# NVIDIA/makani

Hardware: NVIDIA H100
Metric: SFNO-block fwd+bwd samples/sec (higher is better)
Workload: dtype tf32

## Files before the change

### makani_b200/csrc/dft.cu

```cuda
#include "umma_common.cuh"
#include "wgmma_tf32.cuh"
#include "dft_math.cuh"
#include <cmath>
#include <cstdlib>
#include <vector>

namespace b200sht {

int umma_available();

constexpr int kDftMaxHalf = 95;
constexpr int kDftSynWorkers = 10;
constexpr int kDftSynThreads = 32 * (kDftSynWorkers + 2);
constexpr int kDftSynStages = 4;
__host__ __device__ constexpr int dft_out_box(int N2) {
  int d = N2 < 32 ? N2 : 32;
  while (N2 % d != 0) --d;
  return 8 * d;
}

struct DftTables {
  float* et;
  float* eb;
  float2* tw;
  float* zeros;
  int N2, half, M2, nkb;
};

bool dft_shape_ok(int nlon, int mmax) {
  if (nlon % 8 != 0) return false;
  const int N2 = nlon / 8;
  return N2 >= 2 && N2 / 2 <= kDftMaxHalf && (mmax + 7) / 8 <= 32 && mmax <= nlon / 2 + 1;
}

__global__ void dft_tables_kernel(float* et, float* eb, float2* tw, int N2, int half, int M2, int nkb, int nlon) {
  const int i = blockIdx.x * blockDim.x + threadIdx.x;
  if (i < 2 * 128 * 32) {
    const int m2 = i % 32, row = i / 32, p = (row >> 3) & 1, j2 = 8 * (row >> 4) + (row & 7);
    float v = 0.f;
    if (j2 <= half && m2 < M2) {
      const long long t = ((long long)m2 * j2) % N2;
      const double ang = 2.0 * M_PI * (double)t / (double)N2;
      v = tf32_rn((float)(p == 0 ? cos(ang) : sin(ang)));
    }
    et[i] = v;
  }
  if (i < nkb * 2 * 32 * 32) {
    const int jl = i % 32, m2 = (i / 32) % 32, p = (i / 1024) % 2, kb = i / 2048;
    const int j2 = kb * 32 + jl;
    float v = 0.f;
    if (j2 <= half && m2 < M2) {
      const long long t = ((long long)m2 * j2) % N2;
      const double ang = 2.0 * M_PI * (double)t / (double)N2;
      v = tf32_rn((float)(p == 0 ? cos(ang) : sin(ang)));
      if (2 * j2 == N2) v *= 0.5f;
    }
    eb[i] = v;
  }
  if (i < 8 * N2) {
    const int j2 = i % N2, c = i / N2;
    const double ang = 2.0 * M_PI * (double)(c * j2) / (double)nlon;
    tw[i] = make_float2((float)cos(ang), (float)sin(ang));
  }
}

int dft_plan_init(Plan* pl) {
  pl->dft_state = nullptr;
  if (!umma_available()) return -1;
  if (!dft_shape_ok(pl->nlon, pl->mmax)) return -1;
  DftTables* t = new DftTables();
  t->N2 = pl->nlon / 8; t->half = t->N2 / 2; t->M2 = (pl->mmax + 7) / 8;
  t->nkb = (t->half + 1 + 31) / 32;
  t->et = nullptr; t->eb = nullptr; t->tw = nullptr; t->zeros = nullptr;
  const size_t neb = (size_t)t->nkb * 2 * 32 * 32;
  cudaError_t e = cudaMalloc(&t->et, sizeof(float) * 2 * 128 * 32);
  if (e == cudaSuccess) e = cudaMalloc(&t->eb, sizeof(float) * neb);
  if (e == cudaSuccess) e = cudaMalloc(&t->tw, sizeof(float2) * 8 * t->N2);
  if (e == cudaSuccess) e = cudaMalloc(&t->zeros, sizeof(float) * 8 * t->N2);
  if (e == cudaSuccess) e = cudaMemset(t->zeros, 0, sizeof(float) * 8 * t->N2);
  if (e == cudaSuccess) {
    const int n = 8192 > 8 * t->N2 ? 8192 : 8 * t->N2;
    dft_tables_kernel<<<(n + 255) / 256, 256>>>(t->et, t->eb, t->tw, t->N2, t->half, t->M2, t->nkb, pl->nlon);
    e = cudaGetLastError();
    if (e == cudaSuccess) e = cudaStreamSynchronize(0);
  }
  if (e != cudaSuccess) {
    cudaFree(t->et); cudaFree(t->eb); cudaFree(t->tw); cudaFree(t->zeros);
    delete t;
    return -1;
  }
  pl->dft_state = t;
  return 0;
}

void dft_plan_destroy(Plan* pl) {
  DftTables* t = static_cast<DftTables*>(pl->dft_state);
  if (!t) return;
  cudaFree(t->et); cudaFree(t->eb); cudaFree(t->tw); cudaFree(t->zeros);
  delete t;
  pl->dft_state = nullptr;
}

static bool dft_enabled() {
  static const int on = [] { const char* e = getenv("B200SHT_DFT"); return e ? atoi(e) : 1; }();
  return on != 0;
}
bool dft_usable(const Plan* pl) { return pl->dft_state != nullptr && dft_enabled(); }

static unsigned long long* g_dft_prof = nullptr;
static unsigned long long* dft_prof_buffer() {
  static const int on = [] { const char* e = getenv("B200SHT_DFT_PROF"); return e ? atoi(e) : 0; }();
  if (!on) return nullptr;
  if (!g_dft_prof) {
    if (cudaMalloc(&g_dft_prof, 16 * sizeof(unsigned long long)) != cudaSuccess) { g_dft_prof = nullptr; return nullptr; }
    cudaMemset(g_dft_prof, 0, 16 * sizeof(unsigned long long));
  }
  return g_dft_prof;
}
int dft_profile_read(unsigned long long* out16) {
  if (!g_dft_prof) { for (int i = 0; i < 16; ++i) out16[i] = 0; return 0; }
  B200_CHECK_CUDA(cudaDeviceSynchronize());
  B200_CHECK_CUDA(cudaMemcpy(out16, g_dft_prof, 16 * sizeof(unsigned long long), cudaMemcpyDeviceToHost));
  B200_CHECK_CUDA(cudaMemset(g_dft_prof, 0, 16 * sizeof(unsigned long long)));
  return 0;
}
#ifdef B200SHT_DFT_PROFILE
constexpr bool kDftProfile = true;
#else
constexpr bool kDftProfile = false;
#endif
__device__ __forceinline__ void prof_wait(unsigned long long* prof, int slot, uint64_t* bar, uint32_t parity, bool lead) {
  if (!kDftProfile || prof == nullptr) { mbar_wait(bar, parity); return; }
  const long long t0 = clock64();
  mbar_wait(bar, parity);
  if (lead) atomicAdd(prof + slot, (unsigned long long)(clock64() - t0));
}
__device__ __forceinline__ void prof_wait_nocall(unsigned long long* prof, int slot, uint64_t* bar, uint32_t parity, bool lead) {
  if (!kDftProfile || prof == nullptr) { mbar_wait_nocall(bar, parity); return; }
  const long long t0 = clock64();
  mbar_wait_nocall(bar, parity);
  if (lead) atomicAdd(prof + slot, (unsigned long long)(clock64() - t0));
}

static int make_tmap_out(CUtensorMap* tm, void* base, bool bf16, int nlon, int nlat, long long rows, int ow) {
  TmapKey key;
  memset(&key, 0, sizeof(key));
  key.base = base; key.rank = 3; key.kind = bf16 ? 7 : 6;
  key.dims[0] = nlon; key.dims[1] = nlat; key.dims[2] = rows; key.box[0] = ow;
  int slot = 0;
  if (tmap_lookup(key, tm, &slot)) return 0;
  PFN_encodeTiled enc = get_encode();
  if (!enc) { set_error("cuTensorMapEncodeTiled is unavailable"); return B200SHT_ERR_UNSUPPORTED; }
  static thread_local bool ctx_bound = false;
  if (!ctx_bound) { cudaFree(nullptr); ctx_bound = true; }
  const int es = bf16 ? 2 : 4;
  cuuint64_t gd[3] = {(cuuint64_t)nlon, (cuuint64_t)nlat, (cuuint64_t)rows};
  cuuint64_t gst[2] = {(cuuint64_t)nlon * es, (cuuint64_t)nlon * nlat * es};
  cuuint32_t bx[3] = {(cuuint32_t)ow, 8, 1}, el[3] = {1, 1, 1};
  if (gst[0] % 16 != 0 || (reinterpret_cast<uintptr_t>(base) & 15) != 0 || (ow * es) % 16 != 0) {
    set_error("tensor map (output): base / row pitch / box row not 16-byte aligned");
    return B200SHT_ERR_INVALID;
  }
  CUresult r = enc(tm, bf16 ? CU_TENSOR_MAP_DATA_TYPE_BFLOAT16 : CU_TENSOR_MAP_DATA_TYPE_FLOAT32, 3, base, gd, gst, bx, el,
                   CU_TENSOR_MAP_INTERLEAVE_NONE, CU_TENSOR_MAP_SWIZZLE_NONE, CU_TENSOR_MAP_L2_PROMOTION_L2_256B, CU_TENSOR_MAP_FLOAT_OOB_FILL_NONE);
  if (r != CUDA_SUCCESS) { set_error("cuTensorMapEncodeTiled (output) failed (%d)", (int)r); return B200SHT_ERR_CUDA; }
  tmap_store(key, tm, slot);
  return 0;
}

template <typename T> __device__ __forceinline__ void st_out(T* p, float v);
template <> __device__ __forceinline__ void st_out<float>(float* p, float v) { *p = v; }
template <> __device__ __forceinline__ void st_out<__nv_bfloat16>(__nv_bfloat16* p, float v) { *p = __float2bfloat16_rn(v); }
template <typename T> __device__ __forceinline__ uint32_t ld_raw(const T* p);
template <> __device__ __forceinline__ uint32_t ld_raw<float>(const float* p) { return __float_as_uint(__ldg(p)); }
template <> __device__ __forceinline__ uint32_t ld_raw<__nv_bfloat16>(const __nv_bfloat16* p) { return (uint32_t)__ldg(reinterpret_cast<const unsigned short*>(p)); }

#ifndef B200_DFT_TF32_MODE
#define B200_DFT_TF32_MODE 2
#endif
constexpr float kTruncComp = 1.0f + 0.0009765625f / 3.0f;
__device__ __forceinline__ float tf32_operand(float v) {
#if B200_DFT_TF32_MODE == 0
  return tf32_rn(v);
#elif B200_DFT_TF32_MODE == 1
  return __uint_as_float((__float_as_uint(v) + 0x1000u) & 0xffffe000u);
#else
  return v;
#endif
}
__device__ __forceinline__ float tf32_operand_unscaled(float v) {
#if B200_DFT_TF32_MODE == 2
  return v * kTruncComp;
#else
  return tf32_operand(v);
#endif
}

__device__ __forceinline__ pr pr_operand(pr v) { return make_pr(tf32_operand(v.v.x), tf32_operand(v.v.y)); }
__device__ __forceinline__ pr pr_operand_unscaled(pr v) {
#if B200_DFT_TF32_MODE == 2
  return rmul(v, kTruncComp);
#else
  return pr_operand(v);
#endif
}

template <typename T> __device__ __forceinline__ float ld_in(const T* p);
template <> __device__ __forceinline__ float ld_in<float>(const float* p) { return __ldg(p); }
template <> __device__ __forceinline__ float ld_in<__nv_bfloat16>(const __nv_bfloat16* p) {
  return __uint_as_float((uint32_t)__ldg(reinterpret_cast<const unsigned short*>(p)) << 16);
}

struct DftSynParams {
  alignas(64) CUtensorMap tmZ;
  alignas(64) CUtensorMap tmE;
  alignas(64) CUtensorMap tmY;
  const float* Z;
  const float2* tw;
  const float* rowscale;
  const float* bias;
  unsigned long long* prof;
  int R, C, nlat, nlon, kp, mmax, N2, half, M2, mode, ntiles, ktiles, has_nyq, ow;
};

template <typename T>
__global__ void __launch_bounds__(kDftSynThreads, 1) dft_synthesis_kernel(const __grid_constant__ DftSynParams p) {
  extern __shared__ uint8_t smem_raw[];
  __shared__ unsigned long long prof_s[16];
  unsigned long long* const prof = (kDftProfile && p.prof) ? prof_s : nullptr;
  if (kDftProfile && threadIdx.x < 16) prof_s[threadIdx.x] = 0;
  const uint32_t raw = smem_u32(smem_raw);
  const uint32_t base = (raw + 1023u) & ~1023u;
  uint8_t* gbase = smem_raw + (base - raw);
  const int N2 = p.N2;
  const int nlon = 8 * N2;
  const int ow = p.ow;
  const uint32_t obytes = (8u * nlon * sizeof(T) + 1023u) & ~1023u;
  const uint32_t sA = base, sB = base + 32768, sO = sB + kDftSynStages * 16384;
  T* const outS = reinterpret_cast<T*>(gbase + (sO - base));
  float2* tws = reinterpret_cast<float2*>(gbase + (sO - base) + 2 * obytes);
  int* oofs = reinterpret_cast<int*>(reinterpret_cast<uint8_t*>(tws) + ((8 * N2 * 8 + 15) & ~15));
  uint64_t* bars = reinterpret_cast<uint64_t*>(reinterpret_cast<uint8_t*>(oofs) + 8 * N2 * 4);
  uint64_t* full = bars;
  uint64_t* empty = full + kDftSynStages;
  uint64_t* e_full = empty + kDftSynStages;
  uint64_t* staged = e_full + 1;
  uint64_t* ofree = staged + 2;

  const int warp = __shfl_sync(0xffffffffu, (int)(threadIdx.x >> 5), 0), lane = threadIdx.x & 31;
  pdl_trigger();
  const int nblk = (p.half + 8) / 8;
  const int nwork = kDftSynWorkers < 2 * nblk ? kDftSynWorkers : 2 * nblk;
  const bool is_tma = (warp == kDftSynWorkers), is_store = (warp == kDftSynWorkers + 1);

  if (threadIdx.x == 0) {
    for (int s = 0; s < kDftSynStages; ++s) { mbar_init(&full[s], 1); mbar_init(&empty[s], nblk); }
    mbar_init(e_full, 1);
    for (int b = 0; b < 2; ++b) { mbar_init(&staged[b], 32 * nblk); mbar_init(&ofree[b], 1); }
    fence_barrier_init();
    prefetch_tmap(&p.tmZ);
    prefetch_tmap(&p.tmE);
    prefetch_tmap(&p.tmY);
  }
  for (int i = threadIdx.x; i < 8 * p.N2; i += blockDim.x) tws[i] = p.tw[i];
  for (int i = threadIdx.x; i < 8 * N2; i += blockDim.x) {
    const int j = N2 * (i & 7) + (i >> 3);
    oofs[i] = (j / ow) * 8 * ow + j % ow;
  }
  __syncthreads();
  const long long t_cta0 = (kDftProfile && p.prof && threadIdx.x == 0) ? clock64() : 0;
  pdl_wait();

  if (is_tma) {
    if (lane == 0) {
      mbar_expect_tx(e_full, 32768);
      tma_load_2d(sA, &p.tmE, e_full, 0, 0);
      tma_load_2d(sA + 16384, &p.tmE, e_full, 0, 128);
      int n = 0;
      for (int ti = blockIdx.x; ti < p.ntiles; ti += gridDim.x, ++n) {
        const int s = n % kDftSynStages, it = n / kDftSynStages;
        if (it > 0) prof_wait(prof, 8, &empty[s], (it - 1) & 1, true);
        mbar_expect_tx(&full[s], 16384);
        const uint32_t st = sB + s * 16384;
        tma_load_5d(st, &p.tmZ, &full[s], 0, 0, 0, 0, ti);
        tma_load_5d(st + 4096, &p.tmZ, &full[s], 0, 1, 0, 0, ti);
        tma_load_5d(st + 8192, &p.tmZ, &full[s], 0, 0, 0, 1, ti);
        tma_load_5d(st + 12288, &p.tmZ, &full[s], 0, 1, 0, 1, ti);
      }
    }
    __syncwarp();
  } else if (is_store) {
    if (lane == 0) {
      int n = 0;
      for (int ti = blockIdx.x; ti < p.ntiles; ti += gridDim.x, ++n) {
        const int b = n & 1;
        prof_wait(prof, 11, &staged[b], (n >> 1) & 1, true);
        const int r = ti / p.ktiles, k0 = (ti - r * p.ktiles) * 8;
        if (k0 < p.nlat)
          for (int bx = 0; bx * ow < nlon; ++bx) tma_store_3d(&p.tmY, sO + b * obytes + bx * 8 * ow * (uint32_t)sizeof(T), bx * ow, k0, r);
        bulk_commit();
        bulk_wait_read0();
        mbar_arrive(&ofree[b]);
      }
      bulk_wait0();
    }
    __syncwarp();
  } else {
    const int kpi = lane & 3;
    const bool n2odd = (N2 & 1) != 0;
    const float smul = p.mode == 0 ? 2.f : 1.f;
    const int nyq_m = nlon / 2;
    const uint8_t* const gE = gbase;
    uint32_t zoff[2][4];
#pragma unroll
    for (int h = 0; h < 2; ++h)
#pragma unroll
      for (int cc = 0; cc < 4; ++cc) zoff[h][cc] = swz128((uint32_t)((kpi + 4 * h) * 128 + (8 * cc + (lane >> 2)) * 4));
    mbar_wait(e_full, 0);
    for (int task = warp; warp < nwork; task += nwork) {
      const int n = task / nblk, blk = task - n * nblk;
      const int ti = blockIdx.x + n * gridDim.x;
      if (ti >= p.ntiles) break;
      const int r = ti / p.ktiles, k0 = (ti - r * p.ktiles) * 8;
      const int ka = k0 + 2 * kpi;
      const int s = n % kDftSynStages, it = n / kDftSynStages;
      float rsa = 1.f, rsb = 1.f, z0a = 0.f, z0b = 0.f, zna = 0.f, znb = 0.f;
      if (p.mode == 1) {
        const float2 rs = *reinterpret_cast<const float2*>(p.rowscale + ka);
        rsa = rs.x; rsb = rs.y;
      } else {
        const float* zt = p.Z + (size_t)ti * 2 * p.M2 * 64 + 2 * kpi;
        const float2 z0 = *reinterpret_cast<const float2*>(zt);
        z0a = z0.x; z0b = z0.y;
        if (p.has_nyq) {
          const float2 zn = *reinterpret_cast<const float2*>(zt + (nyq_m >> 3) * 64 + (nyq_m & 7) * 8);
          zna = zn.x; znb = zn.y;
        }
      }
      const float bias = p.bias ? __ldg(p.bias + r % p.C) : 0.f;
      const pr sc = make_pr(smul * rsa, smul * rsb);
      const pr off_e = make_pr(bias - rsa * (z0a + zna), bias - rsb * (z0b + znb));
      const pr off_o = make_pr(bias - rsa * (z0a - zna), bias - rsb * (z0b - znb));
      prof_wait(prof, 9, &full[s], it & 1, lane == 0);
      if (prof && lane == 0) atomicAdd(prof + 13, 1ull);
      float acc[2][8][4];
#pragma unroll
      for (int a = 0; a < 2; ++a)
#pragma unroll
        for (int c = 0; c < 8; ++c) acc[a][c][0] = acc[a][c][1] = acc[a][c][2] = acc[a][c][3] = 0.f;
      {
        const uint8_t* const zs = gbase + 32768 + (size_t)s * 16384;
#pragma unroll
        for (int kk = 0; kk < 32; kk += 8) {
          uint32_t fa[4];
          frag_a<false>(gE, 16 * blk, kk, fa);
#pragma unroll
          for (int c = 0; c < 8; ++c) {
            const uint8_t* const zc = zs + (c >> 2) * 4096 + kk * 128;
            const uint32_t zr[2] = {*reinterpret_cast<const uint32_t*>(zc + zoff[0][c & 3]), *reinterpret_cast<const uint32_t*>(zc + zoff[1][c & 3])};
            const uint32_t zi[2] = {*reinterpret_cast<const uint32_t*>(zc + 8192 + zoff[0][c & 3]),
                                    *reinterpret_cast<const uint32_t*>(zc + 8192 + zoff[1][c & 3])};
            mma_tf32(acc[0][c], fa, zr);
            mma_tf32(acc[1][c], fa, zi);
          }
        }
      }
      __syncwarp();
      if (lane == 0) mbar_arrive(&empty[s]);
      {
        const int j2 = 8 * blk + (lane >> 2);
        const bool valid = j2 <= p.half;
        const bool paired = valid && j2 != 0 && 2 * j2 != N2;
        const int jp = N2 - j2;
        float2 tw[8], tp[8];
        tw[0] = make_float2(1.f, 0.f);
#pragma unroll
        for (int c = 1; c < 8; ++c) tw[c] = valid ? tws[c * N2 + j2] : make_float2(1.f, 0.f);
        dft_partner_twiddles(tw, tp);
        T* const ob = outS + (size_t)(n & 1) * (obytes / sizeof(T)) + 2 * kpi * ow;
        if (n >= 2) prof_wait(prof, 10, &ofree[n & 1], ((n >> 1) - 1) & 1, lane == 0);
        {
          pr vr[8], vi[8], x[8];
#pragma unroll
          for (int c = 0; c < 8; ++c) {
            vr[c] = make_pr(acc[0][c][0], acc[0][c][1]) - make_pr(acc[1][c][2], acc[1][c][3]);
            vi[c] = make_pr(acc[0][c][2], acc[0][c][3]) + make_pr(acc[1][c][0], acc[1][c][1]);
          }
          dft_syn_radix8<pr>(vr, vi, tw, x);
          const pr o0 = (j2 & 1) ? off_o : off_e, o1 = (j2 & 1) ? off_e : off_o;
          const int4* const op = reinterpret_cast<const int4*>(oofs + 8 * (valid ? j2 : 0));
          const int4 oa = op[0], ob4 = op[1];
          const int of[8] = {oa.x, oa.y, oa.z, oa.w, ob4.x, ob4.y, ob4.z, ob4.w};
#pragma unroll
          for (int j1 = 0; j1 < 8; ++j1) {
            const pr o = rfma(x[j1], sc, (n2odd && (j1 & 1)) ? o1 : o0);
            if (valid) { st_out<T>(ob + of[j1], o.v.x); st_out<T>(ob + of[j1] + ow, o.v.y); }
          }
        }
        {
          pr vr[8], vi[8], x[8];
#pragma unroll
          for (int c = 0; c < 8; ++c) {
            vr[c] = make_pr(acc[0][c][0], acc[0][c][1]) + make_pr(acc[1][c][2], acc[1][c][3]);
            vi[c] = make_pr(acc[1][c][0], acc[1][c][1]) - make_pr(acc[0][c][2], acc[0][c][3]);
          }
          dft_syn_radix8<pr>(vr, vi, tp, x);
          const pr o0 = (jp & 1) ? off_o : off_e, o1 = (jp & 1) ? off_e : off_o;
          const int4* const op = reinterpret_cast<const int4*>(oofs + 8 * (paired ? jp : 0));
          const int4 oa = op[0], ob4 = op[1];
          const int of[8] = {oa.x, oa.y, oa.z, oa.w, ob4.x, ob4.y, ob4.z, ob4.w};
#pragma unroll
          for (int j1 = 0; j1 < 8; ++j1) {
            const pr o = rfma(x[j1], sc, (n2odd && (j1 & 1)) ? o1 : o0);
            if (paired) { st_out<T>(ob + of[j1], o.v.x); st_out<T>(ob + of[j1] + ow, o.v.y); }
          }
        }
        fence_proxy_async();
        mbar_arrive(&staged[n & 1]);
      }
    }
  }
  __syncthreads();
  if (kDftProfile && p.prof && threadIdx.x == 0) prof_s[12] = (unsigned long long)(clock64() - t_cta0);
  if (kDftProfile) __syncthreads();
  if (kDftProfile && p.prof && threadIdx.x < 16) atomicAdd(p.prof + threadIdx.x, prof_s[threadIdx.x]);
}

int dft_synthesis(const Plan* pl, const float* Z, void* y, int dtype, int B, int C, const float* bias, int mode, cudaStream_t st) {
  const DftTables* t = static_cast<const DftTables*>(pl->dft_state);
  B200_REQUIRE(t != nullptr, "dft_synthesis: plan has no DFT tables");
  const int R = B * C;
  DftSynParams p;
  memset(&p, 0, sizeof(p));
  p.Z = Z; p.tw = t->tw; p.rowscale = pl->d_rowscale; p.bias = bias; p.prof = dft_prof_buffer();
  p.R = R; p.C = C; p.nlat = pl->nlat; p.nlon = pl->nlon; p.kp = pl->kp; p.mmax = pl->mmax;
  p.N2 = t->N2; p.half = t->half; p.mode = mode;
  p.ktiles = pl->kp / 8; p.ntiles = R * p.ktiles;
  p.has_nyq = (pl->mmax == pl->nlon / 2 + 1) ? 1 : 0;
  p.M2 = t->M2;
  {
    long long d[5] = {32, 2, t->M2, 2, (long long)R * (pl->kp / 8)}, s[5] = {1, 32, 64, (long long)t->M2 * 64, 2ll * t->M2 * 64};
    int bx[5] = {32, 1, 32, 1, 1};
    int rc = make_tmap(&p.tmZ, Z, 5, d, s, bx);
    if (rc) return rc;
  }
  {
    long long d[2] = {32, 256}, s[2] = {1, 32};
    int bx[2] = {32, 128};
    int rc = make_tmap(&p.tmE, t->et, 2, d, s, bx);
    if (rc) return rc;
  }
  const bool bf16 = (dtype == B200SHT_BF16);
  p.ow = dft_out_box(t->N2);
  {
    int rc = make_tmap_out(&p.tmY, y, bf16, pl->nlon, pl->nlat, R, p.ow);
    if (rc) return rc;
  }
  const size_t obytes = (8 * (size_t)pl->nlon * (bf16 ? 2 : 4) + 1023) & ~(size_t)1023;
  const size_t smem = 1024 + 32768 + (size_t)kDftSynStages * 16384 + 2 * obytes + ((8 * (size_t)t->N2 * 8 + 15) & ~(size_t)15) +
                      8 * (size_t)t->N2 * 4 + (2 * kDftSynStages + 5) * 8;
  const int sms = usable_sms(pl->sm_count > 0 ? pl->sm_count : 132);
  const int ctas = p.ntiles < sms ? p.ntiles : sms;
#define B200_LAUNCH_SYN(TT)                                                                                          \
  do {                                                                                                                \
    struct Tag {};                                                                                                    \
    B200_CHECK_CUDA((ensure_dynamic_smem<Tag>(dft_synthesis_kernel<TT>, smem)));                                     \
    B200_CHECK_CUDA(launch_pdl(dft_synthesis_kernel<TT>, dim3(ctas), dim3(kDftSynThreads), smem, st, p));            \
  } while (0)
  if (bf16) { B200_LAUNCH_SYN(__nv_bfloat16); } else { B200_LAUNCH_SYN(float); }
#undef B200_LAUNCH_SYN
  B200_CHECK_LAUNCH();
  return 0;
}

__host__ __device__ constexpr int dft_box_group(int N2, int es) { return (N2 * es) % 16 == 0 ? 1 : (2 * N2 * es) % 16 == 0 ? 2 : (4 * N2 * es) % 16 == 0 ? 4 : 8; }

static int make_tmap_segments(CUtensorMap* tm, const void* base, bool bf16, int nlon, int gs, long long rows, int box_cols) {
  TmapKey key;
  memset(&key, 0, sizeof(key));
  key.base = base; key.rank = 3; key.kind = bf16 ? 5 : 4;
  key.dims[0] = nlon; key.dims[1] = gs; key.dims[2] = rows; key.box[0] = box_cols;
  int slot = 0;
  if (tmap_lookup(key, tm, &slot)) return 0;
  PFN_encodeTiled enc = get_encode();
  if (!enc) { set_error("cuTensorMapEncodeTiled is unavailable"); return B200SHT_ERR_UNSUPPORTED; }
  static thread_local bool ctx_bound = false;
  if (!ctx_bound) { cudaFree(nullptr); ctx_bound = true; }
  const int es = bf16 ? 2 : 4, N2 = nlon / 8;
  cuuint64_t gd[3] = {(cuuint64_t)gs * N2, (cuuint64_t)(8 / gs), (cuuint64_t)rows};
  cuuint64_t gst[2] = {(cuuint64_t)gs * N2 * es, (cuuint64_t)nlon * es};
  cuuint32_t bx[3] = {(cuuint32_t)box_cols, (cuuint32_t)(8 / gs), 16}, el[3] = {1, 1, 1};
  if (gst[0] % 16 != 0 || gst[1] % 16 != 0 || (reinterpret_cast<uintptr_t>(base) & 15) != 0 || (box_cols * es) % 16 != 0) {
    set_error("tensor map (segments): base / pitch / box row not 16-byte aligned");
    return B200SHT_ERR_INVALID;
  }
  CUresult r = enc(tm, bf16 ? CU_TENSOR_MAP_DATA_TYPE_BFLOAT16 : CU_TENSOR_MAP_DATA_TYPE_FLOAT32, 3, const_cast<void*>(base), gd, gst, bx, el,
                   CU_TENSOR_MAP_INTERLEAVE_NONE, CU_TENSOR_MAP_SWIZZLE_NONE, CU_TENSOR_MAP_L2_PROMOTION_L2_256B, CU_TENSOR_MAP_FLOAT_OOB_FILL_NONE);
  if (r != CUDA_SUCCESS) { set_error("cuTensorMapEncodeTiled (segments) failed (%d)", (int)r); return B200SHT_ERR_CUDA; }
  tmap_store(key, tm, slot);
  return 0;
}

constexpr int kDftAnaStages = 2;
constexpr int kDftAnaMma = 8, kDftAnaLoader = 8, kDftAnaProd0 = 9, kDftAnaThreads = 544;

struct DftAnaParams {
  alignas(64) CUtensorMap tmB;
  alignas(64) CUtensorMap tmXc;
  alignas(64) CUtensorMap tmXp;
  float* X;
  const float2* tw;
  const float* rowscale;
  unsigned long long* prof;
  int R, nlat, nlon, kp, mmax, N2, half, M2, nkb, mode, ntiles, ktiles, nraw, gs;
};

template <typename T, int N2T>
__global__ void __launch_bounds__(kDftAnaThreads, 1) dft_analysis_kernel(const __grid_constant__ DftAnaParams p) {
  extern __shared__ uint8_t smem_raw[];
  __shared__ unsigned long long prof_s[16];
  unsigned long long* const prof = (kDftProfile && p.prof) ? prof_s : nullptr;
  if (kDftProfile && threadIdx.x < 16) prof_s[threadIdx.x] = 0;
  const uint32_t raw = smem_u32(smem_raw);
  const uint32_t base = (raw + 1023u) & ~1023u;
  uint8_t* gbase = smem_raw + (base - raw);
  constexpr int kAl = 16 / (int)sizeof(T);
  constexpr int kWc = (sizeof(T) == 2) ? 40 : 32, kWp = (sizeof(T) == 2) ? 40 : 36;
  constexpr uint32_t kColBytes = 16u * kWc * sizeof(T), kParBytes = 16u * kWp * sizeof(T);
  constexpr uint32_t kRawBytes = 8u * (kColBytes + kParBytes);
  const uint32_t oB = 0, oA = 3 * 8192, oR = oA + kDftAnaStages * 65536, oT = oR + (uint32_t)p.nraw * kRawBytes, oBar = oT + 3 * 7 * 32 * 8;
  const uint32_t sBm = base + oB, sAr = base + oA, sRaw = base + oR;
  uint8_t* gA = gbase + oA;
  const uint8_t* gR = gbase + oR;
  float2* twS = reinterpret_cast<float2*>(gbase + oT);
  uint64_t* full = reinterpret_cast<uint64_t*>(gbase + oBar);
  uint64_t* empty = full + kDftAnaStages;
  uint64_t* raw_full = empty + kDftAnaStages;
  uint64_t* raw_empty = raw_full + 4;
  uint64_t* b_full = raw_empty + 4;

  const int warp = __shfl_sync(0xffffffffu, (int)(threadIdx.x >> 5), 0), lane = threadIdx.x & 31;
  pdl_trigger();
  const int nkb = p.nkb;
  const int N2 = N2T > 0 ? N2T : p.N2;
  const int gs = N2T > 0 ? dft_box_group(N2T, (int)sizeof(T)) : p.gs;
  for (int i = threadIdx.x; i < nkb * 7 * 32; i += blockDim.x) {
    const int ln = i & 31, c = (i >> 5) % 7 + 1, kb = i / 224;
    const int j2 = 32 * kb + ln;
    float2 w = (j2 <= p.half) ? p.tw[c * N2 + j2] : make_float2(1.f, 0.f);
#if B200_DFT_TF32_MODE == 2
    w.x *= kTruncComp; w.y *= kTruncComp;
#endif
    twS[i] = w;
  }
  if (threadIdx.x == 0) {
    for (int s = 0; s < kDftAnaStages; ++s) { mbar_init(&full[s], 8 * 32); mbar_init(&empty[s], kDftAnaMma); }
    for (int s = 0; s < p.nraw; ++s) { mbar_init(&raw_full[s], 1); mbar_init(&raw_empty[s], 8); }
    mbar_init(b_full, 1);
    fence_barrier_init();
    prefetch_tmap(&p.tmB);
    prefetch_tmap(&p.tmXc);
    prefetch_tmap(&p.tmXp);
  }
  for (int i = threadIdx.x; i < kDftAnaStages * 2 * 512; i += blockDim.x) {
    const int st = i >> 10, pl = (i >> 9) & 1, off = i & 511;
    reinterpret_cast<float*>(gA + (size_t)st * 65536)[(pl ? 12288 : 4096) + off] = 0.f;
  }
  fence_proxy_async();
  __syncthreads();
  const long long t_cta0 = (kDftProfile && p.prof && threadIdx.x == 0) ? clock64() : 0;
  pdl_wait();

  if (warp == kDftAnaLoader) {
    if (lane == 0) {
      mbar_expect_tx(b_full, (uint32_t)nkb * 8192);
      for (int kb = 0; kb < nkb; ++kb) {
        tma_load_2d(sBm + kb * 8192, &p.tmB, b_full, 0, kb * 64);
        tma_load_2d(sBm + kb * 8192 + 4096, &p.tmB, b_full, 0, kb * 64 + 32);
      }
      int n = 0;
      for (int ti = blockIdx.x; ti < p.ntiles; ti += gridDim.x, ++n) {
        const int r = ti / p.ktiles, row0 = r * p.nlat + (ti - r * p.ktiles) * 16;
        for (int kb = 0; kb < nkb; ++kb) {
          const int g = n * nkb + kb, rs = g % p.nraw, it = g / p.nraw;
          if (it > 0) prof_wait_nocall(prof, 2, &raw_empty[rs], (it - 1) & 1, true);
          mbar_expect_tx(&raw_full[rs], kRawBytes);
          const uint32_t dst = sRaw + rs * kRawBytes;
#pragma unroll
          for (int gm = 0; gm < 8; ++gm) {
            if (gm >= gs) break;
            const int sc = N2 * gm + 32 * kb, sp = N2 * gm + N2 - 32 * kb - 31;
            tma_load_3d(dst + gm * (8 / gs) * kColBytes, &p.tmXc, &raw_full[rs], (sc / kAl) * kAl, 0, row0);
            tma_load_3d(dst + 8 * kColBytes + gm * (8 / gs) * kParBytes, &p.tmXp, &raw_full[rs], sp < 0 ? 0 : (sp / kAl) * kAl, 0, row0);
          }
        }
      }
    }
    __syncwarp();
  } else if (warp < kDftAnaMma) {
    const size_t plane = (size_t)p.R * p.kp;
    const int c = warp, gq = lane >> 2, q = lane & 3;
    const uint32_t aw = sAr + (uint32_t)(warp >> 2) * 8192;
    mbar_wait_nocall(b_full, 0);
    int n = 0;
    for (int ti = blockIdx.x; ti < p.ntiles; ti += gridDim.x, ++n) {
      const int r = ti / p.ktiles, k0 = (ti - r * p.ktiles) * 16;
      float acc[8][4];
      int prev = 0;
      for (int kb = 0; kb < nkb; ++kb) {
        const int g = n * nkb + kb, s = g % kDftAnaStages, it = g / kDftAnaStages;
        prof_wait_nocall(prof, 3, &full[s], it & 1, lane == 0);
        const uint32_t a0 = aw + (uint32_t)s * 65536;
        const uint64_t d_er = wgmma_desc_kmajor(a0), d_ei = wgmma_desc_kmajor(a0 + 16384);
        const uint64_t d_or = wgmma_desc_kmajor(a0 + 32768), d_oi = wgmma_desc_kmajor(a0 + 49152);
        const uint64_t d_c = wgmma_desc_kmajor(sBm + kb * 8192), d_s = wgmma_desc_kmajor(sBm + kb * 8192 + 4096);
        wgmma_fence();
#pragma unroll
        for (int k = 0; k < 4; ++k) {
          const int sd = (kb > 0 || k > 0) ? 1 : 0;
          wgmma_tf32<32, 1, 8, 0>(acc, d_er + 2 * k, d_c + 2 * k, sd);
          wgmma_tf32<32, 1, 8, 4>(acc, d_ei + 2 * k, d_c + 2 * k, sd);
          wgmma_tf32<32, 1, 8, 0>(acc, d_oi + 2 * k, d_s + 2 * k, 1);
          wgmma_tf32<32, -1, 8, 4>(acc, d_or + 2 * k, d_s + 2 * k, 1);
        }
        wgmma_commit();
        wgmma_wait<1>();
        if (kb > 0 && lane == 0) mbar_arrive(&empty[prev]);
        prev = s;
      }
      wgmma_wait<0>();
      wgmma_fence_operands(acc);
      if (lane == 0) mbar_arrive(&empty[prev]);
      if (prof && lane == 0) atomicAdd(prof + 5, 1ull);
#pragma unroll
      for (int h = 0; h < 2; ++h) {
        const int k = k0 + gq + 8 * h;
        if (k >= p.kp) continue;
        const float rs = (p.mode == 0) ? ((k < p.nlat) ? __ldg(p.rowscale + k) : 0.f) : 1.f;
        float* xb = p.X + (size_t)r * p.kp + k;
#pragma unroll
        for (int j = 0; j < 4; ++j)
#pragma unroll
          for (int e = 0; e < 2; ++e) {
            const int m = c + 8 * (8 * j + 2 * q + e);
            if (m >= p.mmax) continue;
            const float sc = ((p.mode == 0) ? rs : ((m == 0 || 2 * m == p.nlon) ? 1.f : 2.f)) * kTruncComp;
            float* dst = xb + (size_t)m * 2 * plane;
            dst[0] = __uint_as_float(__float_as_uint(acc[j][2 * h + e] * sc) & 0xffffe000u);
            dst[plane] = __uint_as_float(__float_as_uint(acc[4 + j][2 * h + e] * sc) & 0xffffe000u);
          }
      }
    }
  } else {
    const int pw = warp - kDftAnaProd0;
    constexpr int nprod = kDftAnaThreads / 32 - kDftAnaProd0;
    static_assert(nprod >= 1 && nprod <= 8, "every producer warp must take an item of every K-block (8 items each)");
    constexpr bool kBf16 = (sizeof(T) == 2);
    const T* const rawS = reinterpret_cast<const T*>(gR);
    int n = 0;
    for (int ti = blockIdx.x; ti < p.ntiles; ti += gridDim.x, ++n) {
      const int r = ti / p.ktiles, kt16 = (ti - r * p.ktiles) * 16;
      for (int item = pw; item < 8 * nkb; item += nprod) {
        const int kb = item >> 3, q = item & 7;
        const int k0 = kt16 + 2 * q;
        const int g = n * nkb + kb;
        const int j2 = 32 * kb + lane;
        const int rs = g % p.nraw;
        prof_wait_nocall(prof, 0, &raw_full[rs], (g / p.nraw) & 1, lane == 0);
        if (prof && lane == 0) atomicAdd(prof + 7, 1ull);
        const T* const rb = rawS + (size_t)rs * (kRawBytes / sizeof(T));
        pr xa[8], xb[8];
#pragma unroll
        for (int j1 = 0; j1 < 8; ++j1) {
          const int gm = j1 % gs, ga = j1 / gs, npb = 8 / gs;
          const int sc = N2 * gm + 32 * kb, sp = N2 * gm + N2 - 32 * kb - 31;
          const int ic = sc - (sc / kAl) * kAl + lane;
          int ip = N2 * gm + N2 - j2 - (sp < 0 ? 0 : (sp / kAl) * kAl);
          ip = ip < 0 ? 0 : (ip > kWp - 1 ? kWp - 1 : ip);
          const T* b0 = rb + gm * (16 * npb * kWc) + (2 * q) * (npb * kWc) + ga * kWc;
          const T* b1 = rb + 8 * (16 * kWc) + gm * (16 * npb * kWp) + (2 * q) * (npb * kWp) + ga * kWp;
          const int rowc = npb * kWc, rowp = npb * kWp;
          if constexpr (kBf16) {
            xa[j1] = make_pr(__uint_as_float((uint32_t)reinterpret_cast<const unsigned short*>(b0)[ic] << 16),
                             __uint_as_float((uint32_t)reinterpret_cast<const unsigned short*>(b0)[rowc + ic] << 16));
            xb[j1] = make_pr(__uint_as_float((uint32_t)reinterpret_cast<const unsigned short*>(b1)[ip] << 16),
                             __uint_as_float((uint32_t)reinterpret_cast<const unsigned short*>(b1)[rowp + ip] << 16));
          } else {
            xa[j1] = make_pr(reinterpret_cast<const float*>(b0)[ic], reinterpret_cast<const float*>(b0)[rowc + ic]);
            xb[j1] = make_pr(reinterpret_cast<const float*>(b1)[ip], reinterpret_cast<const float*>(b1)[rowp + ip]);
          }
        }
        if (kb == 0) {
#pragma unroll
          for (int j1 = 0; j1 < 8; ++j1) xb[j1] = (lane == 0) ? make_pr(0.f, 0.f) : xb[j1];
        }
        if (k0 + 1 >= p.nlat) {
          const bool row0ok = k0 < p.nlat;
#pragma unroll
          for (int j1 = 0; j1 < 8; ++j1) {
            xa[j1] = make_pr(row0ok ? xa[j1].v.x : 0.f, 0.f);
            xb[j1] = make_pr(row0ok ? xb[j1].v.x : 0.f, 0.f);
          }
        }
        pr er[8], ei[8], br[8], bi[8];
        float2 tw[8], tp[8];
        tw[0] = make_float2(1.f, 0.f);
        const float2* const twl = twS + kb * 224 + lane;
#pragma unroll
        for (int c = 1; c < 8; ++c) tw[c] = twl[(c - 1) * 32];
        dft_partner_twiddles(tw, tp);
        dft_ana_radix8<pr>(xa, tw, er, ei);
        dft_ana_radix8<pr>(xb, tp, br, bi);
        __syncwarp();
        if (lane == 0) mbar_arrive(&raw_empty[rs]);
        const int s = g % kDftAnaStages, it = g / kDftAnaStages;
        if (it > 0) prof_wait_nocall(prof, 1, &empty[s], (it - 1) & 1, lane == 0);
        float* const stg = reinterpret_cast<float*>(gA + (size_t)s * 65536);
        const int kr0 = 2 * q;
        float* const d0 = stg + kr0 * 32 + ((((lane >> 2) ^ (kr0 & 7)) << 2) | (lane & 3));
        float* const d1 = stg + (kr0 + 1) * 32 + ((((lane >> 2) ^ ((kr0 + 1) & 7)) << 2) | (lane & 3));
#pragma unroll
        for (int c = 0; c < 8; ++c) {
          pr ye_r = er[c] + br[c], yo_r = er[c] - br[c];
          if (c == 0) { ye_r = pr_operand_unscaled(ye_r); yo_r = pr_operand_unscaled(yo_r); }
          else { ye_r = pr_operand(ye_r); yo_r = pr_operand(yo_r); }
          d0[c * 512] = ye_r.v.x; d1[c * 512] = ye_r.v.y;
          d0[8192 + c * 512] = yo_r.v.x; d1[8192 + c * 512] = yo_r.v.y;
          if (c != 0) {
            const pr ye_i = pr_operand(ei[c] + bi[c]), yo_i = pr_operand(ei[c] - bi[c]);
            d0[4096 + c * 512] = ye_i.v.x; d1[4096 + c * 512] = ye_i.v.y;
            d0[12288 + c * 512] = yo_i.v.x; d1[12288 + c * 512] = yo_i.v.y;
          }
        }
        fence_proxy_async();
        mbar_arrive(&full[s]);
      }
    }
  }
  __syncthreads();
  if (kDftProfile && p.prof && threadIdx.x == 0) prof_s[6] = (unsigned long long)(clock64() - t_cta0);
  if (kDftProfile) __syncthreads();
  if (kDftProfile && p.prof && threadIdx.x < 16) atomicAdd(p.prof + threadIdx.x, prof_s[threadIdx.x]);
}

int dft_analysis(const Plan* pl, const void* x, int dtype, int B, int C, float* X, int mode, cudaStream_t st) {
  const DftTables* t = static_cast<const DftTables*>(pl->dft_state);
  B200_REQUIRE(t != nullptr, "dft_analysis: plan has no DFT tables");
  const int R = B * C;
  DftAnaParams p;
  memset(&p, 0, sizeof(p));
  p.X = X; p.tw = t->tw; p.rowscale = pl->d_rowscale; p.prof = dft_prof_buffer();
  p.R = R; p.nlat = pl->nlat; p.nlon = pl->nlon; p.kp = pl->kp; p.mmax = pl->mmax;
  p.N2 = t->N2; p.half = t->half; p.M2 = t->M2; p.nkb = t->nkb; p.mode = mode;
  p.ktiles = (pl->kp + 15) / 16; p.ntiles = R * p.ktiles;
  const bool bf16 = (dtype == B200SHT_BF16);
  p.nraw = bf16 ? 3 : 2;
  {
    long long d[2] = {32, (long long)t->nkb * 64}, s[2] = {1, 32};
    int bx[2] = {32, 32};
    int rc = make_tmap(&p.tmB, t->eb, 2, d, s, bx);
    if (rc) return rc;
  }
  B200_REQUIRE(bf16 || t->N2 % 4 == 0, "dft_analysis: fp32 input needs nlon %% 32 == 0 (16-byte aligned TMA boxes)");
// ... 116 lines not shown
```

Measured before the change: 853.6.

## Pre-permute DFT synthesis operands in shared memory for vectorized MMA fragment loads

The E matrix is now loaded by plain global reads into a fragment-ordered shared layout, and the TMA warp rearranges each staged Z tile so workers fetch MMA B fragments with single 16-byte loads. A new per-stage 'ready' barrier sits between the TMA arrival and the worker compute. Twiddles are packed as float4, output offsets are precomputed in bytes with paired bf16 conversion, and integer divides are replaced by magic-number fast division. The aim is fewer shared-memory load instructions and less index arithmetic in the inner loop. In exchange the producer warp does extra shuffling work and there is one more synchronisation stage per tile.

```diff
diff --git a/makani_b200/csrc/dft.cu b/makani_b200/csrc/dft.cu
--- a/makani_b200/csrc/dft.cu
+++ b/makani_b200/csrc/dft.cu
@@ -17,6 +17,20 @@
   int d = N2 < 32 ? N2 : 32;
   while (N2 % d != 0) --d;
   return 8 * d;
+}
+
+struct FastDiv {
+  uint32_t m, s;
+  int d;
+  __device__ __forceinline__ int div(int n) const { return (int)((__umulhi((uint32_t)n, m) + (uint32_t)n) >> s); }
+};
+static FastDiv make_fastdiv(int d) {
+  FastDiv f;
+  f.d = d;
+  f.s = 0;
+  while ((1ll << f.s) < d) ++f.s;
+  f.m = (uint32_t)((((1ull << 32) * ((1ull << f.s) - (unsigned long long)d)) / (unsigned long long)d) + 1);
+  return f;
 }
 
 struct DftTables {
@@ -168,9 +182,16 @@
   return 0;
 }
 
-template <typename T> __device__ __forceinline__ void st_out(T* p, float v);
-template <> __device__ __forceinline__ void st_out<float>(float* p, float v) { *p = v; }
-template <> __device__ __forceinline__ void st_out<__nv_bfloat16>(__nv_bfloat16* p, float v) { *p = __float2bfloat16_rn(v); }
+template <typename T> __device__ __forceinline__ void st_out2(uint8_t* p0, uint8_t* p1, float a, float b);
+template <> __device__ __forceinline__ void st_out2<float>(uint8_t* p0, uint8_t* p1, float a, float b) {
+  *reinterpret_cast<float*>(p0) = a;
+  *reinterpret_cast<float*>(p1) = b;
+}
+template <> __device__ __forceinline__ void st_out2<__nv_bfloat16>(uint8_t* p0, uint8_t* p1, float a, float b) {
+  const __nv_bfloat162 v = __floats2bfloat162_rn(a, b);
+  *reinterpret_cast<__nv_bfloat16*>(p0) = v.x;
+  *reinterpret_cast<__nv_bfloat16*>(p1) = v.y;
+}
 template <typename T> __device__ __forceinline__ uint32_t ld_raw(const T* p);
 template <> __device__ __forceinline__ uint32_t ld_raw<float>(const float* p) { return __float_as_uint(__ldg(p)); }
 template <> __device__ __forceinline__ uint32_t ld_raw<__nv_bfloat16>(const __nv_bfloat16* p) { return (uint32_t)__ldg(reinterpret_cast<const unsigned short*>(p)); }
@@ -213,15 +234,19 @@
 
 struct DftSynParams {
   alignas(64) CUtensorMap tmZ;
-  alignas(64) CUtensorMap tmE;
   alignas(64) CUtensorMap tmY;
   const float* Z;
+  const float* et;
   const float2* tw;
   const float* rowscale;
   const float* bias;
   unsigned long long* prof;
-  int R, C, nlat, nlon, kp, mmax, N2, half, M2, mode, ntiles, ktiles, has_nyq, ow;
+  FastDiv ktiles, C;
+  int R, nlat, nlon, kp, mmax, N2, half, M2, mode, ntiles, has_nyq, ow;
 };
+
+__host__ __device__ constexpr int syn_kslot(int s, int q, int hi) { return 8 * q + 4 * (s >> 1) + ((2 * (s & 1) + hi + q) & 3); }
+__device__ __forceinline__ uint32_t syn_unit(int g, int q) { return (uint32_t)(8 * (g >> 1) + 4 * ((g ^ (g >> 2)) & 1) + q); }
 
 template <typename T>
 __global__ void __launch_bounds__(kDftSynThreads, 1) dft_synthesis_kernel(const __grid_constant__ DftSynParams p) {
@@ -236,15 +261,15 @@
   const int nlon = 8 * N2;
   const int ow = p.ow;
   const uint32_t obytes = (8u * nlon * sizeof(T) + 1023u) & ~1023u;
-  const uint32_t sA = base, sB = base + 32768, sO = sB + kDftSynStages * 16384;
+  const uint32_t sB = base + 32768, sO = sB + kDftSynStages * 16384;
   T* const outS = reinterpret_cast<T*>(gbase + (sO - base));
-  float2* tws = reinterpret_cast<float2*>(gbase + (sO - base) + 2 * obytes);
-  int* oofs = reinterpret_cast<int*>(reinterpret_cast<uint8_t*>(tws) + ((8 * N2 * 8 + 15) & ~15));
+  float4* tws = reinterpret_cast<float4*>(gbase + (sO - base) + 2 * obytes);
+  int* oofs = reinterpret_cast<int*>(reinterpret_cast<uint8_t*>(tws) + 8 * N2 * 8);
   uint64_t* bars = reinterpret_cast<uint64_t*>(reinterpret_cast<uint8_t*>(oofs) + 8 * N2 * 4);
   uint64_t* full = bars;
-  uint64_t* empty = full + kDftSynStages;
-  uint64_t* e_full = empty + kDftSynStages;
-  uint64_t* staged = e_full + 1;
+  uint64_t* ready = full + kDftSynStages;
+  uint64_t* empty = ready + kDftSynStages;
+  uint64_t* staged = empty + kDftSynStages;
   uint64_t* ofree = staged + 2;
 
   const int warp = __shfl_sync(0xffffffffu, (int)(threadIdx.x >> 5), 0), lane = threadIdx.x & 31;
@@ -254,48 +279,106 @@
   const bool is_tma = (warp == kDftSynWorkers), is_store = (warp == kDftSynWorkers + 1);
 
   if (threadIdx.x == 0) {
-    for (int s = 0; s < kDftSynStages; ++s) { mbar_init(&full[s], 1); mbar_init(&empty[s], nblk); }
-    mbar_init(e_full, 1);
+    for (int s = 0; s < kDftSynStages; ++s) { mbar_init(&full[s], 1); mbar_init(&ready[s], 32); mbar_init(&empty[s], nblk); }
     for (int b = 0; b < 2; ++b) { mbar_init(&staged[b], 32 * nblk); mbar_init(&ofree[b], 1); }
     fence_barrier_init();
     prefetch_tmap(&p.tmZ);
-    prefetch_tmap(&p.tmE);
     prefetch_tmap(&p.tmY);
   }
-  for (int i = threadIdx.x; i < 8 * p.N2; i += blockDim.x) tws[i] = p.tw[i];
+  {
+    constexpr int kEt4 = 16 * 2 * 8 * 32 / 4, kPer = (kEt4 + kDftSynThreads - 1) / kDftSynThreads;
+    float4 ev[kPer];
+#pragma unroll
+    for (int k = 0; k < kPer; ++k) {
+      const int i = threadIdx.x + k * kDftSynThreads;
+      if (i < kEt4) ev[k] = __ldg(reinterpret_cast<const float4*>(p.et) + i);
+    }
+#pragma unroll
+    for (int k = 0; k < kPer; ++k) {
+      const int i = threadIdx.x + k * kDftSynThreads;
+      if (i >= kEt4) continue;
+      const int row = i >> 3, b = row >> 4, cs = (row >> 3) & 1, g = row & 7;
+      const float v[4] = {ev[k].x, ev[k].y, ev[k].z, ev[k].w};
+#pragma unroll
+      for (int e = 0; e < 4; ++e) {
+        const int m2 = 4 * (i & 7) + e, q = m2 >> 3, r = m2 & 7, u = ((r & 3) - q) & 3;
+        const int s = 2 * (r >> 2) + (u >> 1), hi = u & 1;
+        reinterpret_cast<float*>(gbase)[((b * 4 + s) * 32 + 4 * g + q) * 4 + 2 * hi + cs] = v[e];
+      }
+    }
+  }
+  for (int i = threadIdx.x; i < 4 * N2; i += blockDim.x) {
+    const int j2 = i >> 2, c = 2 * (i & 3);
+    tws[i] = make_float4(p.tw[c * N2 + j2].x, p.tw[c * N2 + j2].y, p.tw[(c + 1) * N2 + j2].x, p.tw[(c + 1) * N2 + j2].y);
+  }
   for (int i = threadIdx.x; i < 8 * N2; i += blockDim.x) {
     const int j = N2 * (i & 7) + (i >> 3);
-    oofs[i] = (j / ow) * 8 * ow + j % ow;
+    oofs[i] = ((j / ow) * 8 * ow + j % ow) * (int)sizeof(T);
   }
   __syncthreads();
   const long long t_cta0 = (kDftProfile && p.prof && threadIdx.x == 0) ? clock64() : 0;
   pdl_wait();
 
   if (is_tma) {
-    if (lane == 0) {
-      mbar_expect_tx(e_full, 32768);
-      tma_load_2d(sA, &p.tmE, e_full, 0, 0);
-      tma_load_2d(sA + 16384, &p.tmE, e_full, 0, 128);
-      int n = 0;
-      for (int ti = blockIdx.x; ti < p.ntiles; ti += gridDim.x, ++n) {
-        const int s = n % kDftSynStages, it = n / kDftSynStages;
-        if (it > 0) prof_wait(prof, 8, &empty[s], (it - 1) & 1, true);
-        mbar_expect_tx(&full[s], 16384);
-        const uint32_t st = sB + s * 16384;
-        tma_load_5d(st, &p.tmZ, &full[s], 0, 0, 0, 0, ti);
-        tma_load_5d(st + 4096, &p.tmZ, &full[s], 0, 1, 0, 0, ti);
-        tma_load_5d(st + 8192, &p.tmZ, &full[s], 0, 0, 0, 1, ti);
-        tma_load_5d(st + 12288, &p.tmZ, &full[s], 0, 1, 0, 1, ti);
-      }
-    }
-    __syncwarp();
+    const int ntl = blockIdx.x < p.ntiles ? (p.ntiles - 1 - blockIdx.x) / gridDim.x + 1 : 0;
+    auto load = [&](int n) {
+      const int s = n % kDftSynStages, it = n / kDftSynStages;
+      if (it > 0) prof_wait(prof, 8, &empty[s], (it - 1) & 1, true);
+      mbar_expect_tx(&full[s], 16384);
+      const uint32_t st = sB + s * 16384;
+      const int ti = blockIdx.x + n * gridDim.x;
+      tma_load_5d(st, &p.tmZ, &full[s], 0, 0, 0, 0, ti);
+      tma_load_5d(st + 4096, &p.tmZ, &full[s], 0, 1, 0, 0, ti);
+      tma_load_5d(st + 8192, &p.tmZ, &full[s], 0, 0, 0, 1, ti);
+      tma_load_5d(st + 12288, &p.tmZ, &full[s], 0, 1, 0, 1, ti);
+    };
+    const int q = lane & 3, b = (lane >> 2) & 1, t = lane >> 3;
+    uint32_t src[2][4], dst[2][4];
+#pragma unroll
+    for (int pass = 0; pass < 2; ++pass) {
+      const int h = b ^ pass;
+#pragma unroll
+      for (int i = 0; i < 4; ++i) {
+        src[pass][i] = swz128((uint32_t)((8 * q + 4 * h + ((i + q) & 3)) * 128 + (2 * t + b) * 16));
+        dst[pass][i] = (uint32_t)(t * 1024 + h * 512) + 16 * syn_unit(4 * b + i, q);
+      }
+    }
+    if (lane == 0 && ntl > 0) load(0);
+    for (int n = 0; n < ntl; ++n) {
+      if (lane == 0 && n + 1 < ntl) load(n + 1);
+      const int s = n % kDftSynStages;
+      prof_wait(prof, 14, &full[s], (n / kDftSynStages) & 1, lane == 0);
+      uint8_t* const st = gbase + 32768 + s * 16384;
+      float4 v[4][2][4];
+#pragma unroll
+      for (int blk4 = 0; blk4 < 4; ++blk4)
+#pragma unroll
+        for (int pass = 0; pass < 2; ++pass)
+#pragma unroll
+          for (int i = 0; i < 4; ++i) v[blk4][pass][i] = *reinterpret_cast<const float4*>(st + blk4 * 4096 + src[pass][i]);
+      __syncwarp();
+#pragma unroll
+      for (int blk4 = 0; blk4 < 4; ++blk4) {
+        uint8_t* const sb = st + blk4 * 4096;
+        const float4(&w)[2][4] = v[blk4];
+#pragma unroll
+        for (int pass = 0; pass < 2; ++pass) {
+          *reinterpret_cast<float4*>(sb + dst[pass][0]) = make_float4(w[pass][0].x, w[pass][1].x, w[pass][2].x, w[pass][3].x);
+          *reinterpret_cast<float4*>(sb + dst[pass][1]) = make_float4(w[pass][0].y, w[pass][1].y, w[pass][2].y, w[pass][3].y);
+          *reinterpret_cast<float4*>(sb + dst[pass][2]) = make_float4(w[pass][0].z, w[pass][1].z, w[pass][2].z, w[pass][3].z);
+          *reinterpret_cast<float4*>(sb + dst[pass][3]) = make_float4(w[pass][0].w, w[pass][1].w, w[pass][2].w, w[pass][3].w);
+        }
+      }
+      fence_proxy_async();
+      mbar_arrive(&ready[s]);
+    }
   } else if (is_store) {
     if (lane == 0) {
       int n = 0;
       for (int ti = blockIdx.x; ti < p.ntiles; ti += gridDim.x, ++n) {
         const int b = n & 1;
         prof_wait(prof, 11, &staged[b], (n >> 1) & 1, true);
-        const int r = ti / p.ktiles, k0 = (ti - r * p.ktiles) * 8;
+        const int r = p.ktiles.div(ti), k0 = (ti - r * p.ktiles.d) * 8;
         if (k0 < p.nlat)
           for (int bx = 0; bx * ow < nlon; ++bx) tma_store_3d(&p.tmY, sO + b * obytes + bx * 8 * ow * (uint32_t)sizeof(T), bx * ow, k0, r);
         bulk_commit();
@@ -310,18 +393,14 @@
     const bool n2odd = (N2 & 1) != 0;
     const float smul = p.mode == 0 ? 2.f : 1.f;
     const int nyq_m = nlon / 2;
-    const uint8_t* const gE = gbase;
-    uint32_t zoff[2][4];
-#pragma unroll
-    for (int h = 0; h < 2; ++h)
-#pragma unroll
-      for (int cc = 0; cc < 4; ++cc) zoff[h][cc] = swz128((uint32_t)((kpi + 4 * h) * 128 + (8 * cc + (lane >> 2)) * 4));
-    mbar_wait(e_full, 0);
-    for (int task = warp; warp < nwork; task += nwork) {
-      const int n = task / nblk, blk = task - n * nblk;
+    const uint8_t* const zl = gbase + 32768 + syn_unit(lane >> 2, kpi) * 16;
+    const uint4* const al = reinterpret_cast<const uint4*>(gbase) + lane;
+    int n = 0, blk = warp;
+    if (blk >= nblk) { blk -= nblk; ++n; }
+    while (warp < nwork) {
       const int ti = blockIdx.x + n * gridDim.x;
       if (ti >= p.ntiles) break;
-      const int r = ti / p.ktiles, k0 = (ti - r * p.ktiles) * 8;
+      const int r = p.ktiles.div(ti), k0 = (ti - r * p.ktiles.d) * 8;
       const int ka = k0 + 2 * kpi;
       const int s = n % kDftSynStages, it = n / kDftSynStages;
       float rsa = 1.f, rsb = 1.f, z0a = 0.f, z0b = 0.f, zna = 0.f, znb = 0.f;
@@ -337,11 +416,11 @@
           zna = zn.x; znb = zn.y;
         }
       }
-      const float bias = p.bias ? __ldg(p.bias + r % p.C) : 0.f;
+      const float bias = p.bias ? __ldg(p.bias + (r - p.C.div(r) * p.C.d)) : 0.f;
       const pr sc = make_pr(smul * rsa, smul * rsb);
       const pr off_e = make_pr(bias - rsa * (z0a + zna), bias - rsb * (z0b + znb));
       const pr off_o = make_pr(bias - rsa * (z0a - zna), bias - rsb * (z0b - znb));
-      prof_wait(prof, 9, &full[s], it & 1, lane == 0);
+      prof_wait(prof, 9, &ready[s], it & 1, lane == 0);
       if (prof && lane == 0) atomicAdd(prof + 13, 1ull);
       float acc[2][8][4];
 #pragma unroll
@@ -349,19 +428,21 @@
 #pragma unroll
         for (int c = 0; c < 8; ++c) acc[a][c][0] = acc[a][c][1] = acc[a][c][2] = acc[a][c][3] = 0.f;
       {
-        const uint8_t* const zs = gbase + 32768 + (size_t)s * 16384;
-#pragma unroll
-        for (int kk = 0; kk < 32; kk += 8) {
-          uint32_t fa[4];
-          frag_a<false>(gE, 16 * blk, kk, fa);
+        const uint8_t* const zs = zl + s * 16384;
+        const uint4* const ab = al + blk * 128;
+#pragma unroll
+        for (int h = 0; h < 2; ++h) {
+          const uint4 a0 = ab[64 * h], a1 = ab[64 * h + 32];
+          const uint32_t fa0[4] = {a0.x, a0.y, a0.z, a0.w}, fa1[4] = {a1.x, a1.y, a1.z, a1.w};
 #pragma unroll
           for (int c = 0; c < 8; ++c) {
-            const uint8_t* const zc = zs + (c >> 2) * 4096 + kk * 128;
-            const uint32_t zr[2] = {*reinterpret_cast<const uint32_t*>(zc + zoff[0][c & 3]), *reinterpret_cast<const uint32_t*>(zc + zoff[1][c & 3])};
-            const uint32_t zi[2] = {*reinterpret_cast<const uint32_t*>(zc + 8192 + zoff[0][c & 3]),
-                                    *reinterpret_cast<const uint32_t*>(zc + 8192 + zoff[1][c & 3])};
-            mma_tf32(acc[0][c], fa, zr);
-            mma_tf32(acc[1][c], fa, zi);
+            const uint4 zr = *reinterpret_cast<const uint4*>(zs + (c >> 2) * 4096 + (c & 3) * 1024 + h * 512);
+            const uint4 zi = *reinterpret_cast<const uint4*>(zs + 8192 + (c >> 2) * 4096 + (c & 3) * 1024 + h * 512);
+            const uint32_t zr0[2] = {zr.x, zr.y}, zr1[2] = {zr.z, zr.w}, zi0[2] = {zi.x, zi.y}, zi1[2] = {zi.z, zi.w};
+            mma_tf32(acc[0][c], fa0, zr0);
+            mma_tf32(acc[1][c], fa0, zi0);
+            mma_tf32(acc[0][c], fa1, zr1);
+            mma_tf32(acc[1][c], fa1, zi1);
           }
         }
       }
@@ -373,11 +454,18 @@
         const bool paired = valid && j2 != 0 && 2 * j2 != N2;
         const int jp = N2 - j2;
         float2 tw[8], tp[8];
-        tw[0] = make_float2(1.f, 0.f);
-#pragma unroll
-        for (int c = 1; c < 8; ++c) tw[c] = valid ? tws[c * N2 + j2] : make_float2(1.f, 0.f);
+        {
+          const float4* const tr = tws + 4 * (valid ? j2 : 0);
+#pragma unroll
+          for (int i = 0; i < 4; ++i) {
+            const float4 w = tr[i];
+            tw[2 * i] = make_float2(w.x, w.y);
+            tw[2 * i + 1] = make_float2(w.z, w.w);
+          }
+        }
         dft_partner_twiddles(tw, tp);
-        T* const ob = outS + (size_t)(n & 1) * (obytes / sizeof(T)) + 2 * kpi * ow;
+        uint8_t* const ob0 = reinterpret_cast<uint8_t*>(outS) + (n & 1) * obytes + 2 * kpi * ow * (int)sizeof(T);
+        uint8_t* const ob1 = ob0 + ow * (int)sizeof(T);
         if (n >= 2) prof_wait(prof, 10, &ofree[n & 1], ((n >> 1) - 1) & 1, lane == 0);
         {
           pr vr[8], vi[8], x[8];
@@ -394,7 +482,7 @@
 #pragma unroll
           for (int j1 = 0; j1 < 8; ++j1) {
             const pr o = rfma(x[j1], sc, (n2odd && (j1 & 1)) ? o1 : o0);
-            if (valid) { st_out<T>(ob + of[j1], o.v.x); st_out<T>(ob + of[j1] + ow, o.v.y); }
+            if (valid) st_out2<T>(ob0 + of[j1], ob1 + of[j1], o.v.x, o.v.y);
           }
         }
         {
@@ -412,12 +500,15 @@
 #pragma unroll
           for (int j1 = 0; j1 < 8; ++j1) {
             const pr o = rfma(x[j1], sc, (n2odd && (j1 & 1)) ? o1 : o0);
-            if (paired) { st_out<T>(ob + of[j1], o.v.x); st_out<T>(ob + of[j1] + ow, o.v.y); }
+            if (paired) st_out2<T>(ob0 + of[j1], ob1 + of[j1], o.v.x, o.v.y);
           }
         }
         fence_proxy_async();
         mbar_arrive(&staged[n & 1]);
       }
+      blk += nwork;
+      if (blk >= nblk) { blk -= nblk; ++n; }
+      if (blk >= nblk) { blk -= nblk; ++n; }
     }
   }
   __syncthreads();
@@ -432,10 +523,10 @@
   const int R = B * C;
   DftSynParams p;
   memset(&p, 0, sizeof(p));
-  p.Z = Z; p.tw = t->tw; p.rowscale = pl->d_rowscale; p.bias = bias; p.prof = dft_prof_buffer();
-  p.R = R; p.C = C; p.nlat = pl->nlat; p.nlon = pl->nlon; p.kp = pl->kp; p.mmax = pl->mmax;
+  p.Z = Z; p.et = t->et; p.tw = t->tw; p.rowscale = pl->d_rowscale; p.bias = bias; p.prof = dft_prof_buffer();
+  p.R = R; p.C = make_fastdiv(C); p.nlat = pl->nlat; p.nlon = pl->nlon; p.kp = pl->kp; p.mmax = pl->mmax;
   p.N2 = t->N2; p.half = t->half; p.mode = mode;
-  p.ktiles = pl->kp / 8; p.ntiles = R * p.ktiles;
+  p.ktiles = make_fastdiv(pl->kp / 8); p.ntiles = R * (pl->kp / 8);
   p.has_nyq = (pl->mmax == pl->nlon / 2 + 1) ? 1 : 0;
   p.M2 = t->M2;
   {
@@ -444,12 +535,6 @@
     int rc = make_tmap(&p.tmZ, Z, 5, d, s, bx);
     if (rc) return rc;
   }
-  {
-    long long d[2] = {32, 256}, s[2] = {1, 32};
-    int bx[2] = {32, 128};
-    int rc = make_tmap(&p.tmE, t->et, 2, d, s, bx);
-    if (rc) return rc;
-  }
   const bool bf16 = (dtype == B200SHT_BF16);
   p.ow = dft_out_box(t->N2);
   {
@@ -457,8 +542,8 @@
     if (rc) return rc;
   }
   const size_t obytes = (8 * (size_t)pl->nlon * (bf16 ? 2 : 4) + 1023) & ~(size_t)1023;
-  const size_t smem = 1024 + 32768 + (size_t)kDftSynStages * 16384 + 2 * obytes + ((8 * (size_t)t->N2 * 8 + 15) & ~(size_t)15) +
-                      8 * (size_t)t->N2 * 4 + (2 * kDftSynStages + 5) * 8;
+  const size_t smem = 1024 + 32768 + (size_t)kDftSynStages * 16384 + 2 * obytes + 8 * (size_t)t->N2 * 8 + 8 * (size_t)t->N2 * 4 +
+                      (3 * kDftSynStages + 4) * 8;
   const int sms = usable_sms(pl->sm_count > 0 ? pl->sm_count : 132);
   const int ctas = p.ntiles < sms ? p.ntiles : sms;
 #define B200_LAUNCH_SYN(TT)                                                                                          \
```

New measurement: 899.1 (median of 6 runs). 1.05x the previous value.
